# lms-07/LGTEUN

Measured on AMD Instinct MI355X. Metric: train image-pairs/sec, GF-2 4-band 128x128, K=4, bs=32/GPU, higher is better.
Workload: dtype f32 (GEMMs and the local mixer: split 16-bit MFMA -- f16 pairs in the forward FFN, the W2 products of its backward and P V, bf16 triples elsewhere -- fp32 accumulate; fp32-equivalent); 1 GPU; BASELINE configs[1]: C=4, MS 32x32, PAN 128x128, K=4, 32 pairs/GPU, train step = fwd + L1 + bwd + Adam + StepLR tick; mode=faithful, global_batch=32, parallelism=dp1, dropout=True

## Files before the change

### include/lgteun_hip.h

```cpp
#ifndef LGTEUN_HIP_H
#define LGTEUN_HIP_H

#include <stddef.h>
#include <stdint.h>

#ifdef __cplusplus
extern "C" {
#endif

#define LG_TENSORS_SHARED 12
#define LG_TENSORS_PER_STAGE 119

#define LG_FLAG_FAITHFUL 1
#define LG_FLAG_SAVE 2
#define LG_FLAG_DROPOUT 4

#define LG_FLAG_BWD_LGT 8
#define LG_FLAG_BWD_DATA 16

#define LG_FLAG_CHAINED 32

#define LG_FLAG_DEFER_DEAD 64

#define LG_FLAG_STAGEWISE 128
// ... 10 lines not shown
    int32_t precision;
    uint32_t variant;
} lg_config;

#define LG_VAR_FFN_IMPL_MASK 3u
#define LG_VAR_FFN_STRIP 1u
#define LG_VAR_FFN_SAVE_MASK (3u << 2)
#define LG_VAR_FFN_SAVE3 (1u << 2)
#define LG_VAR_FFN_SAVE5 (2u << 2)
#define LG_VAR_FFN_BWD32_PAIR (1u << 4)
#define LG_VAR_FFN_DWBWD_TILE (1u << 5)
#define LG_VAR_ATTN_BWD_R3 (1u << 6)
#define LG_VAR_DSTEP_TILES (1u << 7)
#define LG_VAR_ATTN_FWD_VALU (1u << 8)
#define LG_VAR_FFN_BF16X3 (1u << 9)
#define LG_VAR_FFT_FULL (1u << 10)
#define LG_VAR_FFN_BWD_BF16X3 (1u << 11)
#define LG_VAR_ATTN_BWD_CORE_M (1u << 12)
#define LG_VAR_FFN_XS (1u << 13)
#define LG_VAR_ATTN_BF16X3 (1u << 14)
#define LG_VAR_FFN_H3_RECOMPUTE (1u << 15)
#define LG_VAR_ATTN_BWD_RESTATS (1u << 16)
#define LG_VAR_REDUCE_PER_BLOCK (1u << 17)
#define LG_VAR_ALL 0x3ffffu

typedef struct lg_plan lg_plan;

const char* lg_version(void);
#define LG_ABI_VERSION 2
int32_t lg_abi_version(void);
const char* lg_last_error(void);

int lg_plan_create(const lg_config* cfg, const int64_t* offsets, int32_t n_offsets, lg_plan** out);
void lg_plan_destroy(lg_plan* plan);
int lg_plan_describe(const lg_plan* plan, char* buf, size_t n);
size_t lg_workspace_bytes(const lg_plan* plan, int32_t B, int32_t train);

int lgteun_forward(const lg_plan* plan, const float* params, const float* ms, const float* pan, float* out,
                   void* workspace, size_t workspace_bytes, int32_t B, int32_t flags, uint64_t seed, void* stream);

int lgteun_dead_forward(const lg_plan* plan, const float* params, void* workspace, size_t workspace_bytes, int32_t B, int32_t flags,
                        uint64_t seed, void* stream);

int lgteun_backward(const lg_plan* plan, const float* params, float* grads, const float* ms, const float* pan,
                    const float* dout, void* workspace, size_t workspace_bytes, int32_t B, int32_t flags,
                    uint64_t seed, void* stream);

// ... 103 lines not shown
```

### lgteun_amd/_lib.py

```python
import ctypes
import os
from ctypes import POINTER, c_char_p, c_double, c_float, c_int32, c_int64, c_size_t, c_uint64, c_void_p

_HERE = os.path.dirname(os.path.abspath(__file__))
LIB_PATH = os.environ.get('LGTEUN_HIP_LIB') or os.path.join(_HERE, '_lgteun_hip.so')

LG_FLAG_FAITHFUL = 1
LG_FLAG_SAVE = 2
LG_FLAG_DROPOUT = 4
LG_FLAG_BWD_LGT = 8
LG_FLAG_BWD_DATA = 16
LG_FLAG_CHAINED = 32
LG_FLAG_DEFER_DEAD = 64
LG_FLAG_STAGEWISE = 128
KERNEL_IDS = {n: i for i, n in enumerate(['none', 'ffn1', 'ffn', 'fft', 'attn', 'upfuse', 'down', 'embed', 'tail', 'datastep', 'ffn1_bwd',
                                           'ffn2_bwd', 'fft_bwd', 'attn_bwd', 'wgrad', 'batch', 'scene_gather', 'scene_blend'])}


class LgConfig(ctypes.Structure):
    _fields_ = [('C', c_int32), ('K', c_int32), ('H', c_int32), ('W', c_int32), ('precision', c_int32), ('variant', ctypes.c_uint32)]


LG_VAR_FFN_STRIP = 1
LG_VAR_FFN_SAVE3, LG_VAR_FFN_SAVE5 = 1 << 2, 2 << 2
LG_VAR_FFN_BWD32_PAIR, LG_VAR_FFN_DWBWD_TILE, LG_VAR_ATTN_BWD_R3 = 1 << 4, 1 << 5, 1 << 6
LG_VAR_DSTEP_TILES = 1 << 7
LG_VAR_ATTN_FWD_VALU = 1 << 8
LG_VAR_FFN_BF16X3 = 1 << 9
LG_VAR_FFT_FULL = 1 << 10
LG_VAR_FFN_BWD_BF16X3 = 1 << 11
LG_VAR_ATTN_BWD_CORE_M = 1 << 12
LG_VAR_FFN_XS = 1 << 13
LG_VAR_ATTN_BF16X3 = 1 << 14
LG_VAR_FFN_H3_RECOMPUTE = 1 << 15
LG_VAR_ATTN_BWD_RESTATS = 1 << 16
LG_VAR_REDUCE_PER_BLOCK = 1 << 17
LG_OPT_ADAM, LG_OPT_ADAMW, LG_OPT_SGD, LG_OPT_RMSPROP = 0, 1, 2, 3
LG_OPT_AMSGRAD, LG_OPT_NESTEROV, LG_OPT_CENTERED = 1, 2, 4
LG_DT_U8, LG_DT_U16, LG_DT_F32 = 0, 1, 2
LG_ABI_VERSION = 2


def variant_from_env(env=None):
    env = os.environ if env is None else env
    v = {'strip': LG_VAR_FFN_STRIP, 'tile': 2, 'xp': 3}.get(env.get('LG_FFN_IMPL', ''), 0)
    v |= {'3': LG_VAR_FFN_SAVE3, '5': LG_VAR_FFN_SAVE5}.get(env.get('LG_FFN_SAVE', ''), 0)
    if env.get('LG_FFN_BWD32') == 'pair':
        v |= LG_VAR_FFN_BWD32_PAIR
    if env.get('LG_FFN_DWBWD') == 'tile':
        v |= LG_VAR_FFN_DWBWD_TILE
    if env.get('LG_ATTN_BWD') in ('old', 'r3'):
        v |= LG_VAR_ATTN_BWD_R3
    if env.get('LG_DSTEP') == 'tiles':
        v |= LG_VAR_DSTEP_TILES
    if env.get('LG_ATTN_FWD', '') == 'valu':
        v |= LG_VAR_ATTN_FWD_VALU
    if env.get('LG_FFN_SPLIT', '') == 'bf16x3':
        v |= LG_VAR_FFN_BF16X3
    if env.get('LG_FFT', '') == 'full':
        v |= LG_VAR_FFT_FULL
    if env.get('LG_FFN_BWD_SPLIT', '') == 'bf16x3':
        v |= LG_VAR_FFN_BWD_BF16X3
    if env.get('LG_ATTN_BWD_CORE', '') == 'm':
        v |= LG_VAR_ATTN_BWD_CORE_M
    if env.get('LG_FFN_FWD', '') == 'xs':
        v |= LG_VAR_FFN_XS
    if env.get('LG_ATTN_SPLIT', '') == 'bf16x3':
        v |= LG_VAR_ATTN_BF16X3
    if env.get('LG_FFN_H3', '') == 'recompute':
        v |= LG_VAR_FFN_H3_RECOMPUTE
    if env.get('LG_ATTN_BWD_STATS', '') == 'recompute':
        v |= LG_VAR_ATTN_BWD_RESTATS
    if env.get('LG_REDUCE', '') == 'per_block':
        v |= LG_VAR_REDUCE_PER_BLOCK
    return v


class LgteunHipError(RuntimeError):
    pass


_lib = None

SIGNATURES = {
    'lg_version': (c_char_p, []),
    'lg_abi_version': (c_int32, []),
    'lg_last_error': (c_char_p, []),
    'lg_plan_create': (c_int32, [POINTER(LgConfig), POINTER(c_int64), c_int32, POINTER(c_void_p)]),
    'lg_plan_destroy': (None, [c_void_p]),
    'lg_plan_describe': (c_int32, [c_void_p, c_char_p, c_size_t]),
    'lg_workspace_bytes': (c_size_t, [c_void_p, c_int32, c_int32]),
    'lgteun_forward': (c_int32, [c_void_p, c_void_p, c_void_p, c_void_p, c_void_p, c_void_p, c_size_t, c_int32, c_int32,
                                 c_uint64, c_void_p]),
    'lgteun_backward': (c_int32, [c_void_p, c_void_p, c_void_p, c_void_p, c_void_p, c_void_p, c_void_p, c_size_t, c_int32,
                                  c_int32, c_uint64, c_void_p]),
    'lgteun_dead_forward': (c_int32, [c_void_p, c_void_p, c_void_p, c_size_t, c_int32, c_int32, c_uint64, c_void_p]),
    'lg_l1_loss': (c_int32, [c_void_p, c_void_p, c_void_p, c_void_p, c_int64, c_int64, c_float, c_void_p]),
# ... 76 lines not shown
```

### lgteun_amd/csrc/bwd_kernels.h

```cpp
#pragma once
#include "common.h"

struct WgradArgs {
    const void* Y;
    const void* X;
    float* dW;
    float* db;
    long P;
    int ldy, ldx, ldw;
    int N, K;
    int n_valid, k_valid;
    int ybf, xbf;
    int xgelu;
};
size_t wgrad_slab_floats(int N, int K, long P);
#define PIXEL_PART_WGS 2048
size_t chan_partial_floats(int C, int B, int H, int W);
struct ChanReduce {
    float* dst[14];
    float* dst2[14];
    int stride[14];
    int NK, C, nslices;
    unsigned allc_mask;
};
// ... 107 lines not shown
int launch_tail_bwd(int C, const TailBwdArgs& a, hipStream_t s);

struct EmbedBwdArgs {
    const float* dx;
    const float* z;
    float* dz;
    const float *dww, *dwb, *w, *b, *lng;
    float *d_dww, *d_dwb, *d_lng, *d_lnb;
    float *d_w, *d_b;
    float* part;
    int HW;
    long total;
};
size_t embed_bwd_part_floats(int C);
int launch_embed_bwd(int C, const EmbedBwdArgs& a, hipStream_t s);

struct DownBwdArgs {
    const float* dy;
    float* du;
    const float* dskip;
    float* dx;
    const float* w;
    int B, H, W;
};
int launch_down_bwd_a(int E, const DownBwdArgs& a, hipStream_t s);
int launch_down_bwd_b(int E, const DownBwdArgs& a, hipStream_t s);

struct UpFuseBwdArgs {
    const float* dy;
    float* dt;
    float* dskip;
    float* v;
    float* dxb;
    float* tmp;
    const float *fw, *upw;
    int B, H, W;
};
int launch_upfuse_bwd_a(int E, const UpFuseBwdArgs& a, hipStream_t s);
int launch_upfuse_bwd_b(int E, const UpFuseBwdArgs& a, hipStream_t s);

struct FfnDwBwdArgs {
    const float* dy;
    const void* g3;
    const void* h2;
    void* dh2;
    int hbf;
    int pre;
    const float *w3t;
    const float* dww;
    float *slab_w, *slab_b;
    float *d_dww, *d_dwb;
    int B, h, w;
};
size_t ffn_dw_bwd_slab_floats(int e, int B, int h, int w);
int launch_ffn_dw_bwd(int e, const FfnDwBwdArgs& a, hipStream_t s);
struct Ffn1BwdArgs {
    const void* dh2;
    const void* g1;
    const float* x;
    const float* dy;
    void* dh1;
    float* y2;
// ... 183 lines not shown
```

### lgteun_amd/csrc/k_bwd.hip

```cpp
#include <string.h>

#include "kernels.h"
#include "bwd_kernels.h"
#include "backward.h"

struct BwdBufs {
    float *dzA, *dzB, *gu3, *gs1, *gu1, *gr, *gd3, *gt1, *gd1;
    float *dx[3];
    float *dh2, *dh1, *y2, *do2, *dg, *dym, *cat, *y1, *dqkv;
    float *w3t[5], *w2t[5], *w1t[5], *wsp, *dt, *dskip, *v, *du, *fft_scratch;
    float* slab_arena;
    float* attn_stats;
    float* ffn_scales;
    size_t slab_cap;
    ReduceQueue rq;
    size_t bytes;
};

static size_t dpos_slab_floats() {
    const size_t f = (size_t)ATTN_BWD_F_WGS * ATTN_BWD_F_ROW, r3 = (size_t)512 * 2 * 64 * 64;
    return f > r3 ? f : r3;
}
static void carve_bwd(const lg_plan* plan, int B, void* base, BwdBufs& bb) {
    const lg_config& c = plan->cfg;
// ... 297 lines not shown
    d.part = bb.rq.take(chan_partial_floats(c.C, B, H, W));
    if (!d.part) return -3;
    RC(launch_dw_bwd(0, d, s));
    RC(launch_resample_adj(0, bb.gd1, dz, planes, H, W, 1, s));
    return bb.rq.block_end();
}

static int lgt_bwd(const lg_plan* pl, const float* P, float* G, int st, const NetBufs& nb, BwdBufs& bb, const float* dout,
                   const float* zin, int B, int flags, uint64_t seed, hipStream_t s) {
    const lg_config& c = pl->cfg;
    const int E = 4 * c.C;
    const long P0 = (long)B * c.H * c.W, P1 = P0 / 4;
    const float* posT = nb.posT + (size_t)st * 5 * 2 * 64 * 64;
    float *A = bb.dx[0], *Bf = bb.dx[1], *Cf = bb.dx[2];
    RC(ffn_transposes(pl, P, st, 0, 5, nb, bb, s));
    TailBwdArgs tb;
    tb.dout = dout; tb.x = nb.blk[4].xout; tb.dx = A; tb.dz = bb.dzA; tb.w = P + pl->lgt(st, L_TAILW);
    tb.d_w = G + pl->lgt(st, L_TAILW); tb.d_b = G + pl->lgt(st, L_TAILB);
    tb.HW = c.H * c.W; tb.total = P0; tb.part = bb.rq.take(tail_bwd_part_floats(c.C));
    if (!tb.part) return -3;
    RC(launch_tail_bwd(c.C, tb, s));
    RC(block_bwd(pl, P, G, st, 4, nb.blk[4], bb, posT + 4 * 8192, A, Bf, Cf, B, flags, seed, s));
    RC(block_bwd(pl, P, G, st, 3, nb.blk[3], bb, posT + 3 * 8192, Cf, Bf, A, B, flags, seed, s));
    UpFuseBwdArgs ub;
    ub.dy = A; ub.dt = bb.dt; ub.dskip = bb.dskip; ub.v = bb.v; ub.dxb = Bf; ub.tmp = Cf;
    ub.fw = P + pl->lgt(st, L_FUSEW); ub.upw = P + pl->lgt(st, L_UPW);
    ub.B = B; ub.H = c.H; ub.W = c.W;
    RC(launch_upfuse_bwd_a(E, ub, s));
    RC(wgrad(A, E, nb.t_up, E, G + pl->lgt(st, L_FUSEW), 2 * E, G + pl->lgt(st, L_FUSEB), P0, E, E, E, E, 0, 0, bb, s));
    RC(wgrad(A, E, nb.blk[1].xout, E, G + pl->lgt(st, L_FUSEW) + E, 2 * E, nullptr, P0, E, E, E, E, 0, 0, bb, s));
    RC(launch_upfuse_bwd_b(E, ub, s));
    RC(wgrad(bb.v, E, nb.blk[2].xout, 2 * E, G + pl->lgt(st, L_UPW), 2 * E, G + pl->lgt(st, L_UPB), P1, E, 2 * E, E, 2 * E, 0, 0, bb, s));
    RC(block_bwd(pl, P, G, st, 2, nb.blk[2], bb, posT + 2 * 8192, Bf, Cf, A, B, flags, seed, s));
    DownBwdArgs db;
    db.dy = A; db.du = bb.du; db.dskip = bb.dskip; db.dx = Bf; db.w = P + pl->lgt(st, L_DOWNW);
    db.B = B; db.H = c.H; db.W = c.W;
    RC(launch_down_bwd_a(E, db, s));
    RC(wgrad(A, 2 * E, nb.u_down, E, G + pl->lgt(st, L_DOWNW), E, G + pl->lgt(st, L_DOWNB), P1, 2 * E, E, 2 * E, E, 0, 0, bb, s));
    RC(launch_down_bwd_b(E, db, s));
    RC(block_bwd(pl, P, G, st, 1, nb.blk[1], bb, posT + 1 * 8192, Bf, Cf, A, B, flags, seed, s));
    RC(block_bwd(pl, P, G, st, 0, nb.blk[0], bb, posT + 0 * 8192, A, Bf, Cf, B, flags, seed, s));
    EmbedBwdArgs eb;
    eb.dx = Cf; eb.z = zin; eb.dz = bb.dzA;
    eb.dww = P + pl->lgt(st, L_PE_DWW); eb.dwb = P + pl->lgt(st, L_PE_DWB); eb.w = P + pl->lgt(st, L_PE_W); eb.b = P + pl->lgt(st, L_PE_B);
    eb.lng = P + pl->lgt(st, L_PE_LNG);
    eb.d_dww = G + pl->lgt(st, L_PE_DWW); eb.d_dwb = G + pl->lgt(st, L_PE_DWB);
    eb.d_lng = G + pl->lgt(st, L_PE_LNG); eb.d_lnb = G + pl->lgt(st, L_PE_LNB);
    eb.d_w = G + pl->lgt(st, L_PE_W); eb.d_b = G + pl->lgt(st, L_PE_B);
    eb.HW = c.H * c.W; eb.total = P0; eb.part = bb.rq.take(embed_bwd_part_floats(c.C));
    if (!eb.part) return -3;
    RC(launch_embed_bwd(c.C, eb, s));
    return 0;
}

int op_data_step_bwd(const lg_plan* pl, const float* P, float* G, int st, NetBufs& nb, void* bwd_ws, const float* z_in, const float* pan,
                     const float* g, float* dz, int B, hipStream_t s) {
    BwdBufs bb;
    carve_bwd(pl, B, bwd_ws, bb);
    ReduceQueueScope rqs(bb, s, pl->route.reduce_per_block);
    const int rc = data_step_bwd(pl, P, G, st, nb, bb, z_in, pan, g, dz, B, s);
    const int rc2 = reduce_queue_end();
// ... 51 lines not shown
```

### lgteun_amd/csrc/k_bwd_pixel.hip

```cpp
#include <string.h>

#include "kernels.h"
#include "bwd_kernels.h"
#include "resample_tile.h"

template <int N>
__device__ __forceinline__ float block_sum(float (&v)[N], float* sm ) {
    const int wave = threadIdx.x >> 6, lane = threadIdx.x & 63;
#pragma unroll
    for (int i = 0; i < N; ++i) {
        float s = v[i];
#pragma unroll
        for (int off = 32; off > 0; off >>= 1) s += __shfl_xor(s, off);
        if (lane == 0) sm[wave * N + i] = s;
    }
    __syncthreads();
    float r = 0.f;
    if (threadIdx.x < N) r = sm[threadIdx.x] + sm[N + threadIdx.x] + sm[2 * N + threadIdx.x] + sm[3 * N + threadIdx.x];
    __syncthreads();
    return r;
}

template <int MODE>
__global__ __launch_bounds__(256) void k_resample_adj(const float* __restrict__ gout, float* __restrict__ gin, int hi, int wi, int ho, int wo,
                                                      int accumulate, int rt, int grows) {
    constexpr int NC = AdjPlan<MODE>::NC, PL = NC + 1;
    extern __shared__ float sm[];
// ... 515 lines not shown
    const int ix = (int)(p % a.W);
    const long r = p / a.W;
    const int iy = (int)(r % a.H);
    const long b = r / a.H;
    const int ho = a.H / 2, wo = a.W / 2;
    AdjPlan<0> py, px;
    py.make(iy, a.H, ho);
    px.make(ix, a.W, wo);
    float4 acc = *reinterpret_cast<const float4*>(a.dskip + p * E + 4 * q);
#pragma unroll
    for (int ya = 0; ya < 3; ++ya) {
        const int yy = clampi(py.base + ya, 0, ho - 1);
#pragma unroll
        for (int xb = 0; xb < 3; ++xb) {
            const int xx = clampi(px.base + xb, 0, wo - 1);
            const float wgt = py.coef[ya] * px.coef[xb];
            const float4 v = *reinterpret_cast<const float4*>(a.du + ((b * ho + yy) * (long)wo + xx) * E + 4 * q);
            acc.x += wgt * v.x; acc.y += wgt * v.y; acc.z += wgt * v.z; acc.w += wgt * v.w;
        }
    }
    *reinterpret_cast<float4*>(a.dx + p * E + 4 * q) = acc;
}

int launch_down_bwd_a(int E, const DownBwdArgs& a, hipStream_t s) {
    long total = (long)a.B * (a.H / 2) * (a.W / 2);
    int grid = (int)((total + 255) / 256);
    if (E == 16) k_down_bwd_a<16><<<grid, 256, 0, s>>>(a);
    else if (E == 32) k_down_bwd_a<32><<<grid, 256, 0, s>>>(a);
    else { lg_set_error("down_bwd: E=%d unsupported", E); return -1; }
    LG_CHECK_LAUNCH();
    return 0;
}
int launch_down_bwd_b(int E, const DownBwdArgs& a, hipStream_t s) {
    long total = (long)a.B * a.H * a.W;
    const int ppw = 256 / (E / 4);
    int grid = (int)((total + ppw - 1) / ppw);
    if (E == 16) k_down_bwd_b<16><<<grid, 256, 0, s>>>(a);
    else if (E == 32) k_down_bwd_b<32><<<grid, 256, 0, s>>>(a);
    else { lg_set_error("down_bwd: E=%d unsupported", E); return -1; }
    LG_CHECK_LAUNCH();
    return 0;
}

template <int E>
__global__ __launch_bounds__(256) void k_upfuse_bwd_a(UpFuseBwdArgs a) {
    constexpr int LPP = E / 4, PPW = 256 / LPP, LDU = E + 4;
    __shared__ float sFw[E * 2 * E];
    __shared__ __attribute__((aligned(16))) float dx_[PPW * LDU];
    lds_stage(sFw, a.fw, E * 2 * E);
    __syncthreads();
    const int q = threadIdx.x % LPP, slot = threadIdx.x / LPP;
    const long total = (long)a.B * a.H * a.W;
    for (long p = (long)blockIdx.x * PPW + slot; p < total; p += (long)gridDim.x * PPW) {
        *reinterpret_cast<float4*>(dx_ + slot * LDU + 4 * q) = *reinterpret_cast<const float4*>(a.dy + p * E + 4 * q);
// ... 78 lines not shown
    __builtin_amdgcn_wave_barrier();
    __builtin_amdgcn_fence(__ATOMIC_ACQUIRE, "wavefront");
    float v[E];
#pragma unroll
    for (int k = 0; k < E / 4; ++k) {
        const float4 t = *reinterpret_cast<const float4*>(vx + slot * LDU + 4 * k);
        v[4 * k] = t.x; v[4 * k + 1] = t.y; v[4 * k + 2] = t.z; v[4 * k + 3] = t.w;
    }
    float o[NO];
#pragma unroll
    for (int j = 0; j < NO; ++j) {
        float acc = 0.f;
#pragma unroll
        for (int n = 0; n < E; ++n) acc += sUw[n * 2 * E + NO * q + j] * v[n];
        o[j] = acc;
    }
    if (pv) {
        float4* dxo = reinterpret_cast<float4*>(a.dxb + p * 2 * E + NO * q);
        dxo[0] = make_float4(o[0], o[1], o[2], o[3]);
        dxo[1] = make_float4(o[4], o[5], o[6], o[7]);
    }
}

int launch_upfuse_bwd_a(int E, const UpFuseBwdArgs& a, hipStream_t s) {
    if (E != 16 && E != 32) { lg_set_error("upfuse_bwd: E=%d unsupported", E); return -1; }
    const long total = (long)a.B * a.H * a.W;
    const int ppw = 256 / (E / 4);
    if (total % ppw) { lg_set_error("upfuse_bwd: %ld pixels are not a multiple of %d", total, ppw); return -2; }
    const long ng = total / ppw;
    const int grid = (int)(ng < 2048 ? ng : 2048);
    if (E == 16) k_upfuse_bwd_a<16><<<grid, 256, 0, s>>>(a);
    else k_upfuse_bwd_a<32><<<grid, 256, 0, s>>>(a);
    LG_CHECK_LAUNCH();
    return 0;
}
int launch_upfuse_bwd_b(int E, const UpFuseBwdArgs& a, hipStream_t s) {
    if (!a.tmp) { lg_set_error("upfuse_bwd: row-contracted scratch missing"); return -2; }
    if (E != 16 && E != 32) { lg_set_error("upfuse_bwd: E=%d unsupported", E); return -1; }
    const int ppw = 256 / (E / 4), wi = a.W / 2;
    const int rows = a.B * a.H;
    dim3 gh((wi + ppw - 1) / ppw, rows < 1024 ? rows : 1024);
    if (E == 16) k_upadj_h<16><<<gh, 256, 0, s>>>(a.dt, a.tmp, rows, a.W);
    else k_upadj_h<32><<<gh, 256, 0, s>>>(a.dt, a.tmp, rows, a.W);
    LG_CHECK_LAUNCH();
    const long total = (long)a.B * (a.H / 2) * wi;
    const int grid = (int)((total + ppw - 1) / ppw);
    if (E == 16) k_upfuse_bwd_b<16><<<grid, 256, 0, s>>>(a);
    else k_upfuse_bwd_b<32><<<grid, 256, 0, s>>>(a);
    LG_CHECK_LAUNCH();
    return 0;
}
```

### lgteun_amd/csrc/mfma.h

```cpp
#pragma once
#include <hip/hip_runtime.h>

typedef float f32x4 __attribute__((ext_vector_type(4)));

template <int MT, int NT, int K>
__device__ __forceinline__ void wave_gemm(f32x4 (&acc)[MT][NT], const float* A, int lda, const float* __restrict__ Wg) {
    const int lane = threadIdx.x & 63, r = lane & 15, g = lane >> 4;
#pragma unroll 2
    for (int k0 = 0; k0 < K; k0 += 16) {
        float4 av[MT], bv[NT];
#pragma unroll
        for (int mt = 0; mt < MT; ++mt) av[mt] = *reinterpret_cast<const float4*>(A + (mt * 16 + r) * lda + k0 + 4 * g);
#pragma unroll
        for (int nt = 0; nt < NT; ++nt) bv[nt] = *reinterpret_cast<const float4*>(Wg + (size_t)(nt * 16 + r) * K + k0 + 4 * g);
#pragma unroll
        for (int ks = 0; ks < 4; ++ks)
#pragma unroll
            for (int mt = 0; mt < MT; ++mt)
#pragma unroll
                for (int nt = 0; nt < NT; ++nt) {
                    const float a_ = ks == 0 ? av[mt].x : (ks == 1 ? av[mt].y : (ks == 2 ? av[mt].z : av[mt].w));
                    const float b_ = ks == 0 ? bv[nt].x : (ks == 1 ? bv[nt].y : (ks == 2 ? bv[nt].z : bv[nt].w));
                    acc[mt][nt] = __builtin_amdgcn_mfma_f32_16x16x4f32(a_, b_, acc[mt][nt], 0, 0, 0);
                }
// ... 32 lines not shown
#pragma unroll
        for (int kb = 0; kb < KB; ++kb) bf[nt][kb] = *reinterpret_cast<const float4*>(Wg + (size_t)(nt * 16 + r) * K + kb * 16 + 4 * g);
}
template <int MT, int NT, int KB>
__device__ __forceinline__ void wave_gemm_rb(f32x4 (&acc)[MT][NT], const float* A, int lda, const float4 (&bf)[NT][KB]) {
    const int lane = threadIdx.x & 63, r = lane & 15, g = lane >> 4;
#pragma unroll
    for (int kb = 0; kb < KB; ++kb) {
        float4 av[MT];
#pragma unroll
        for (int mt = 0; mt < MT; ++mt) av[mt] = *reinterpret_cast<const float4*>(A + (mt * 16 + r) * lda + kb * 16 + 4 * g);
#pragma unroll
        for (int ks = 0; ks < 4; ++ks)
#pragma unroll
            for (int mt = 0; mt < MT; ++mt)
#pragma unroll
                for (int nt = 0; nt < NT; ++nt) {
                    const float a_ = ks == 0 ? av[mt].x : (ks == 1 ? av[mt].y : (ks == 2 ? av[mt].z : av[mt].w));
                    const float b_ = ks == 0 ? bf[nt][kb].x : (ks == 1 ? bf[nt][kb].y : (ks == 2 ? bf[nt][kb].z : bf[nt][kb].w));
                    acc[mt][nt] = __builtin_amdgcn_mfma_f32_16x16x4f32(a_, b_, acc[mt][nt], 0, 0, 0);
                }
    }
}
```

### lgteun_amd/csrc/route.h

```cpp
#pragma once
#include <stddef.h>
#include "../../include/lgteun_hip.h"

enum FfnFwdKernel {
    FFN_FWD_XR,
    FFN_FWD_XS,
    FFN_FWD_X32,
    FFN_FWD_X64,
    FFN_FWD_STRIP,
    FFN_FWD_TILE,
    FFN_FWD_UNFUSED
};
enum FfnArith { FFN_ARITH_F32, FFN_ARITH_BF16, FFN_ARITH_F16X2, FFN_ARITH_BF16X3 };
enum FfnSlot { FFN_SLOT_A1 = 1, FFN_SLOT_G1 = 2, FFN_SLOT_H2 = 4, FFN_SLOT_A3 = 8, FFN_SLOT_G3 = 16 };
enum FfnDwBwdKernel { FFN_DWBWD_XS, FFN_DWBWD_H, FFN_DWBWD_TILE };
enum Ffn1BwdKernel { FFN1_BWD_XS, FFN1_BWD_X32, FFN1_BWD_TILE };

struct FfnRoute {
    int e, h, w;
    FfnFwdKernel fwd[2];
    FfnArith arith;
    bool hbf;
    bool scales;
    int wsplit_np;
// ... 3 lines not shown
    FfnDwBwdKernel dw;
    Ffn1BwdKernel px;
    bool bwd_scales;
    bool wgrad_w2, wgrad_w1, wgrad_w3;
};

enum AttnFwdKernel { ATTN_FWD_M, ATTN_FWD_VALU };
enum AttnBwdKernel { ATTN_BWD_F, ATTN_BWD_R3, ATTN_BWD_R3_CORE_M };
struct MixerRoute {
    int e;
    AttnFwdKernel fwd;
    bool bf16;
    bool f16x2;
    bool stats;
    AttnBwdKernel bwd;
};

struct LgRoute {
    FfnRoute ffn[2];
    MixerRoute mix[2];
    bool dstep_fused;
    bool fft_full;
    bool reduce_per_block;
};

int lg_resolve_route(const lg_config& cfg, LgRoute* r);
int lg_describe_route(const lg_config& cfg, const LgRoute& r, char* buf, size_t n);
```

### lgteun_amd/csrc/route.hip

```cpp
#include <stdio.h>

#include "kernels.h"
#include "bwd_kernels.h"

static void resolve_ffn(const lg_config& cfg, int e, int h, int w, FfnRoute& f) {
    const uint32_t v = cfg.variant;
    const int impl = (int)(v & LG_VAR_FFN_IMPL_MASK);
    const uint32_t sv = v & LG_VAR_FFN_SAVE_MASK;
    const bool split = impl == 0;
    const bool strips = (h & 7) == 0 && (w & 15) == 0;
    f.e = e; f.h = h; f.w = w;
    f.hbf = cfg.precision == 1 && e != 64;
    f.scales = cfg.precision == 0 && split && !(v & LG_VAR_FFN_BF16X3);
    f.arith = !split ? FFN_ARITH_F32 : f.hbf ? FFN_ARITH_BF16 : f.scales ? FFN_ARITH_F16X2 : FFN_ARITH_BF16X3;
    f.wsplit_np = e < 32 ? 0 : f.hbf ? 1 : f.scales ? 2 : 3;

    const int save_form = (e != 16 || !split) ? 5 : sv == LG_VAR_FFN_SAVE5 ? 5 : (sv == LG_VAR_FFN_SAVE3 ? (cfg.precision == 0 ? 3 : 5) : 2);
    f.pre = save_form != 5;
    f.px = (e == 16 && save_form == 2) || (e == 32 && split && !(v & LG_VAR_FFN_BWD32_PAIR)) ? FFN1_BWD_XS : (e == 32 && split) ? FFN1_BWD_X32 : FFN1_BWD_TILE;
    const bool dw_tile = (v & LG_VAR_FFN_DWBWD_TILE) && !(e == 16 && f.hbf);
    f.dw = ((e == 16 && save_form == 2) || (e == 32 && split)) && !dw_tile && strips ? FFN_DWBWD_XS : FFN_DWBWD_TILE;
    const bool xr_built = split && !(v & LG_VAR_FFN_XS) && (f.hbf || f.scales);
    if (e == 16 && f.dw == FFN_DWBWD_XS && (v & LG_VAR_FFN_H3_RECOMPUTE) && xr_built && !f.hbf) f.dw = FFN_DWBWD_H;
    f.bwd_scales = f.px == FFN1_BWD_XS && f.dw != FFN_DWBWD_TILE && f.scales && !(v & LG_VAR_FFN_BWD_BF16X3);
// ... 21 lines not shown
    const uint32_t v = cfg.variant;
    m.e = e;
    m.fwd = (v & LG_VAR_ATTN_FWD_VALU) ? ATTN_FWD_VALU : ATTN_FWD_M;
    m.bf16 = cfg.precision == 1;
    m.f16x2 = cfg.precision == 0 && m.fwd == ATTN_FWD_M && !(v & LG_VAR_ATTN_BF16X3) && !(v & LG_VAR_FFN_IMPL_MASK) && !(v & LG_VAR_FFN_BF16X3);
    m.bwd = (attn_bwd_fused(e) && !(v & LG_VAR_ATTN_BWD_R3)) ? ATTN_BWD_F : (e == 32 && (v & LG_VAR_ATTN_BWD_CORE_M)) ? ATTN_BWD_R3_CORE_M : ATTN_BWD_R3;
    m.stats = cfg.precision == 0 && m.fwd == ATTN_FWD_M && !(v & LG_VAR_ATTN_BWD_RESTATS) && m.bwd != ATTN_BWD_R3_CORE_M;
}

int lg_resolve_route(const lg_config& cfg, LgRoute* r) {
    const uint32_t v = cfg.variant;
    if (v & ~LG_VAR_ALL) { lg_set_error("plan_create: unknown variant bits 0x%x", v & ~LG_VAR_ALL); return -2; }
    if ((v & LG_VAR_FFN_SAVE_MASK) == LG_VAR_FFN_SAVE_MASK) { lg_set_error("plan_create: invalid FFN save variant"); return -2; }
    if ((v & LG_VAR_FFN_IMPL_MASK) > LG_VAR_FFN_STRIP) { lg_set_error("plan_create: FFN implementation field (LG_VAR_FFN_IMPL_MASK) = %u: only 0 and LG_VAR_FFN_STRIP exist", v & LG_VAR_FFN_IMPL_MASK); return -2; }
    if (cfg.precision == 1 && (v & LG_VAR_FFN_IMPL_MASK)) { lg_set_error("plan_create: FFN implementation field (LG_VAR_FFN_IMPL_MASK): LG_VAR_FFN_STRIP is an fp32 kernel set, precision = 1 has none"); return -2; }
    const int E = 4 * cfg.C;
    resolve_ffn(cfg, E, cfg.H, cfg.W, r->ffn[0]);
    resolve_ffn(cfg, 2 * E, cfg.H / 2, cfg.W / 2, r->ffn[1]);
    resolve_mixer(cfg, E, r->mix[0]);
    resolve_mixer(cfg, 2 * E, r->mix[1]);
    r->dstep_fused = !(v & LG_VAR_DSTEP_TILES) && dstep_fused_ok(cfg.C, cfg.H, cfg.W);
    r->fft_full = (v & LG_VAR_FFT_FULL) != 0;
    r->reduce_per_block = (v & LG_VAR_REDUCE_PER_BLOCK) != 0;
    return 0;
}

static const char* slots_text(unsigned slots, bool a1_pre, bool a3_pre, char (&buf)[48]) {
    int n = 0;
    buf[0] = 0;
    auto add = [&](unsigned bit, const char* name) { if (slots & bit) n += snprintf(buf + n, sizeof(buf) - n, "%s%s", n ? "," : "", name); };
    add(FFN_SLOT_A1, a1_pre ? "a1:h1" : "a1"); add(FFN_SLOT_G1, "g1"); add(FFN_SLOT_H2, "h2"); add(FFN_SLOT_A3, a3_pre ? "a3:h3" : "a3"); add(FFN_SLOT_G3, "g3");
    return n ? buf : "-";
}

int lg_describe_route(const lg_config& cfg, const LgRoute& r, char* buf, size_t n) {
    static const char* const fwd_names[] = {"k_ffn_xr", "k_ffn_xs", "k_ffn_x32", "k_ffn1_x64+k_ffn2_x64", "k_ffn_strip", "k_ffn_fused", "k_ffn1+k_ffn2"};
    static const char* const arith_names[] = {"f32", "bf16", "f16x2", "bf16x3"};
    static const char* const dw_names[] = {"k_ffn_dw_bwd_xs", "k_ffn_dw_bwd_h", "k_ffn_dw_bwd"};
    static const char* const px_names[] = {"k_ffn1_bwd_xs", "k_ffn1_bwd_x32", "k_ffn1_bwd"};
    static const char* const attn_bwd_names[] = {"k_attn_bwd_f", "k_attn_bwd_core+k_attn_bwd_epi", "k_attn_bwd_core_m+k_attn_bwd_epi"};
    size_t off = 0;
    bool full = false;
    auto put = [&](const char* fmt, auto... a) {
        const int k = snprintf(buf + off, n - off, fmt, a...);
        if (k < 0 || (size_t)k >= n - off) full = true; else off += (size_t)k;
    };
// ... 28 lines not shown
```

Measured before the change: 6553 image-pairs/sec.

## Fuse weight-gradient reductions into LGT transition backward kernels (down, upfuse)

Adds fused backward kernels for the LGT down-sampling and up/fuse transitions. Each kernel computes the data gradient and also accumulates the conv weight and bias gradients per workgroup with fp32 MFMA outer products, then a slab reduction sums the partials. This replaces separate wgrad launches that re-read dy and the conv inputs from global memory. The fused path is the default, the old split path stays behind an env flag, and the cost is extra slab scratch and more complex kernels with wave-level barriers.

Result: no change. 6599 image-pairs/sec, median of 6 (+0.7%).

```diff
diff --git a/include/lgteun_hip.h b/include/lgteun_hip.h
--- a/include/lgteun_hip.h
+++ b/include/lgteun_hip.h
@@ -56,7 +56,8 @@
 #define LG_VAR_FFN_H3_RECOMPUTE (1u << 15)
 #define LG_VAR_ATTN_BWD_RESTATS (1u << 16)
 #define LG_VAR_REDUCE_PER_BLOCK (1u << 17)
-#define LG_VAR_ALL 0x3ffffu
+#define LG_VAR_LGT_TRANS_SPLIT (1u << 21)
+#define LG_VAR_ALL 0x23ffffu
 
 typedef struct lg_plan lg_plan;
 
diff --git a/lgteun_amd/_lib.py b/lgteun_amd/_lib.py
--- a/lgteun_amd/_lib.py
+++ b/lgteun_amd/_lib.py
@@ -35,6 +35,7 @@
 LG_VAR_FFN_H3_RECOMPUTE = 1 << 15
 LG_VAR_ATTN_BWD_RESTATS = 1 << 16
 LG_VAR_REDUCE_PER_BLOCK = 1 << 17
+LG_VAR_LGT_TRANS_SPLIT = 1 << 21
 LG_OPT_ADAM, LG_OPT_ADAMW, LG_OPT_SGD, LG_OPT_RMSPROP = 0, 1, 2, 3
 LG_OPT_AMSGRAD, LG_OPT_NESTEROV, LG_OPT_CENTERED = 1, 2, 4
 LG_DT_U8, LG_DT_U16, LG_DT_F32 = 0, 1, 2
@@ -73,6 +74,8 @@
         v |= LG_VAR_ATTN_BWD_RESTATS
     if env.get('LG_REDUCE', '') == 'per_block':
         v |= LG_VAR_REDUCE_PER_BLOCK
+    if env.get('LG_LGT_TRANS_BWD', '') == 'split':
+        v |= LG_VAR_LGT_TRANS_SPLIT
     return v
 
 
diff --git a/lgteun_amd/csrc/bwd_kernels.h b/lgteun_amd/csrc/bwd_kernels.h
--- a/lgteun_amd/csrc/bwd_kernels.h
+++ b/lgteun_amd/csrc/bwd_kernels.h
@@ -153,8 +153,12 @@
     float* dx;
     const float* w;
     int B, H, W;
-};
+    const float* u = nullptr;
+    float* slab = nullptr;
+};
+size_t trans_bwd_slab_floats(int E);
 int launch_down_bwd_a(int E, const DownBwdArgs& a, hipStream_t s);
+int launch_down_bwd_aw(int E, const DownBwdArgs& a, float* d_w, float* d_b, hipStream_t s);
 int launch_down_bwd_b(int E, const DownBwdArgs& a, hipStream_t s);
 
 struct UpFuseBwdArgs {
@@ -166,9 +170,16 @@
     float* tmp;
     const float *fw, *upw;
     int B, H, W;
+    const float* t_up = nullptr;
+    const float* skip = nullptr;
+    const float* xb = nullptr;
+    float* slab = nullptr;
 };
 int launch_upfuse_bwd_a(int E, const UpFuseBwdArgs& a, hipStream_t s);
 int launch_upfuse_bwd_b(int E, const UpFuseBwdArgs& a, hipStream_t s);
+bool upfuse_bwd_rows_ok(int E, int W);
+int launch_upfuse_bwd_ar(int E, const UpFuseBwdArgs& a, float* d_w, float* d_b, hipStream_t s);
+int launch_upfuse_bwd_bw(int E, const UpFuseBwdArgs& a, int upadj, float* d_w, float* d_b, hipStream_t s);
 
 struct FfnDwBwdArgs {
     const float* dy;
diff --git a/lgteun_amd/csrc/k_bwd.hip b/lgteun_amd/csrc/k_bwd.hip
--- a/lgteun_amd/csrc/k_bwd.hip
+++ b/lgteun_amd/csrc/k_bwd.hip
@@ -343,21 +343,43 @@
     RC(launch_tail_bwd(c.C, tb, s));
     RC(block_bwd(pl, P, G, st, 4, nb.blk[4], bb, posT + 4 * 8192, A, Bf, Cf, B, flags, seed, s));
     RC(block_bwd(pl, P, G, st, 3, nb.blk[3], bb, posT + 3 * 8192, Cf, Bf, A, B, flags, seed, s));
+    const bool fused = !pl->route.lgt_trans_split;
+    const bool rows_ok = fused && upfuse_bwd_rows_ok(E, c.W);
     UpFuseBwdArgs ub;
     ub.dy = A; ub.dt = bb.dt; ub.dskip = bb.dskip; ub.v = bb.v; ub.dxb = Bf; ub.tmp = Cf;
     ub.fw = P + pl->lgt(st, L_FUSEW); ub.upw = P + pl->lgt(st, L_UPW);
     ub.B = B; ub.H = c.H; ub.W = c.W;
-    RC(launch_upfuse_bwd_a(E, ub, s));
-    RC(wgrad(A, E, nb.t_up, E, G + pl->lgt(st, L_FUSEW), 2 * E, G + pl->lgt(st, L_FUSEB), P0, E, E, E, E, 0, 0, bb, s));
-    RC(wgrad(A, E, nb.blk[1].xout, E, G + pl->lgt(st, L_FUSEW) + E, 2 * E, nullptr, P0, E, E, E, E, 0, 0, bb, s));
-    RC(launch_upfuse_bwd_b(E, ub, s));
-    RC(wgrad(bb.v, E, nb.blk[2].xout, 2 * E, G + pl->lgt(st, L_UPW), 2 * E, G + pl->lgt(st, L_UPB), P1, E, 2 * E, E, 2 * E, 0, 0, bb, s));
+    ub.t_up = nb.t_up; ub.skip = nb.blk[1].xout; ub.xb = nb.blk[2].xout;
+    if (rows_ok) {
+        ub.slab = bb.rq.take(trans_bwd_slab_floats(E));
+        if (!ub.slab) return -3;
+        RC(launch_upfuse_bwd_ar(E, ub, G + pl->lgt(st, L_FUSEW), G + pl->lgt(st, L_FUSEB), s));
+    } else {
+        RC(launch_upfuse_bwd_a(E, ub, s));
+        RC(wgrad(A, E, nb.t_up, E, G + pl->lgt(st, L_FUSEW), 2 * E, G + pl->lgt(st, L_FUSEB), P0, E, E, E, E, 0, 0, bb, s));
+        RC(wgrad(A, E, nb.blk[1].xout, E, G + pl->lgt(st, L_FUSEW) + E, 2 * E, nullptr, P0, E, E, E, E, 0, 0, bb, s));
+    }
+    if (fused) {
+        ub.slab = bb.rq.take(trans_bwd_slab_floats(E));
+        if (!ub.slab) return -3;
+        RC(launch_upfuse_bwd_bw(E, ub, rows_ok ? 0 : 1, G + pl->lgt(st, L_UPW), G + pl->lgt(st, L_UPB), s));
+    } else {
+        RC(launch_upfuse_bwd_b(E, ub, s));
+        RC(wgrad(bb.v, E, nb.blk[2].xout, 2 * E, G + pl->lgt(st, L_UPW), 2 * E, G + pl->lgt(st, L_UPB), P1, E, 2 * E, E, 2 * E, 0, 0, bb, s));
+    }
     RC(block_bwd(pl, P, G, st, 2, nb.blk[2], bb, posT + 2 * 8192, Bf, Cf, A, B, flags, seed, s));
     DownBwdArgs db;
     db.dy = A; db.du = bb.du; db.dskip = bb.dskip; db.dx = Bf; db.w = P + pl->lgt(st, L_DOWNW);
     db.B = B; db.H = c.H; db.W = c.W;
-    RC(launch_down_bwd_a(E, db, s));
-    RC(wgrad(A, 2 * E, nb.u_down, E, G + pl->lgt(st, L_DOWNW), E, G + pl->lgt(st, L_DOWNB), P1, 2 * E, E, 2 * E, E, 0, 0, bb, s));
+    if (fused) {
+        db.u = nb.u_down;
+        db.slab = bb.rq.take(trans_bwd_slab_floats(E));
+        if (!db.slab) return -3;
+        RC(launch_down_bwd_aw(E, db, G + pl->lgt(st, L_DOWNW), G + pl->lgt(st, L_DOWNB), s));
+    } else {
+        RC(launch_down_bwd_a(E, db, s));
+        RC(wgrad(A, 2 * E, nb.u_down, E, G + pl->lgt(st, L_DOWNW), E, G + pl->lgt(st, L_DOWNB), P1, 2 * E, E, 2 * E, E, 0, 0, bb, s));
+    }
     RC(launch_down_bwd_b(E, db, s));
     RC(block_bwd(pl, P, G, st, 1, nb.blk[1], bb, posT + 1 * 8192, Bf, Cf, A, B, flags, seed, s));
     RC(block_bwd(pl, P, G, st, 0, nb.blk[0], bb, posT + 0 * 8192, A, Bf, Cf, B, flags, seed, s));
diff --git a/lgteun_amd/csrc/k_bwd_pixel.hip b/lgteun_amd/csrc/k_bwd_pixel.hip
--- a/lgteun_amd/csrc/k_bwd_pixel.hip
+++ b/lgteun_amd/csrc/k_bwd_pixel.hip
@@ -3,6 +3,7 @@
 #include "kernels.h"
 #include "bwd_kernels.h"
 #include "resample_tile.h"
+#include "mfma.h"
 
 template <int N>
 __device__ __forceinline__ float block_sum(float (&v)[N], float* sm ) {
@@ -564,6 +565,76 @@
     *reinterpret_cast<float4*>(a.dx + p * E + 4 * q) = acc;
 }
 
+
+#define TRANS_BWD_WGS 512
+__device__ __forceinline__ float4 keep4(bool keep, const float4& v) { return make_float4(keep ? v.x : 0.f, keep ? v.y : 0.f, keep ? v.z : 0.f, keep ? v.w : 0.f); }
+struct DownAwOps { float4 y0, y1, x0; };
+template <int E>
+__device__ __forceinline__ DownAwOps down_aw_fetch(const DownBwdArgs& a, long p, long total, int q) {
+    const long pc_ = p < total ? p : total - 1;
+    DownAwOps o;
+    o.y0 = *reinterpret_cast<const float4*>(a.dy + pc_ * 2 * E + 8 * q);
+    o.y1 = *reinterpret_cast<const float4*>(a.dy + pc_ * 2 * E + 8 * q + 4);
+    o.x0 = *reinterpret_cast<const float4*>(a.u + pc_ * E + 4 * q);
+    return o;
+}
+template <int E>
+__global__ __launch_bounds__(256) void k_down_bwd_aw(DownBwdArgs a) {
+    constexpr int LPP = E / 4, PPW = 256 / LPP, PY = px_pitch(2 * E), PX = px_pitch(E), MT = 2 * E / 16, NT = E / 16;
+    constexpr int IMG = PPW * (PY + PX), SCR = 4 * wave_pixel_row<MT, NT>();
+    __shared__ float sW[2 * E * E];
+    __shared__ __attribute__((aligned(16))) float sm[IMG > SCR ? IMG : SCR];
+    float* yi = sm;
+    float* xi = sm + PPW * PY;
+    lds_stage(sW, a.w, 2 * E * E);
+    __syncthreads();
+    const int q = threadIdx.x % LPP, slot = threadIdx.x / LPP, wave = threadIdx.x >> 6;
+    const long total = (long)a.B * (a.H / 2) * (a.W / 2);
+    const long ngroups = (total + PPW - 1) / PPW;
+    f32x4 acc[MT][NT];
+    float bsum[MT];
+#pragma unroll
+    for (int mt = 0; mt < MT; ++mt) {
+        bsum[mt] = 0.f;
+#pragma unroll
+        for (int nt = 0; nt < NT; ++nt) acc[mt][nt] = f32x4{0.f, 0.f, 0.f, 0.f};
+    }
+    DownAwOps nx = down_aw_fetch<E>(a, blockIdx.x * (long)PPW + slot, total, q);
+    for (long grp = blockIdx.x; grp < ngroups; grp += gridDim.x) {
+        const long p = grp * PPW + slot;
+        const bool pv = p < total;
+        *reinterpret_cast<float4*>(yi + slot * PY + 8 * q) = keep4(pv, nx.y0);
+        *reinterpret_cast<float4*>(yi + slot * PY + 8 * q + 4) = keep4(pv, nx.y1);
+        *reinterpret_cast<float4*>(xi + slot * PX + 4 * q) = keep4(pv, nx.x0);
+        nx = down_aw_fetch<E>(a, p + (long)gridDim.x * PPW, total, q);
+        __builtin_amdgcn_fence(__ATOMIC_RELEASE, "wavefront");
+        __builtin_amdgcn_wave_barrier();
+        __builtin_amdgcn_fence(__ATOMIC_ACQUIRE, "wavefront");
+        float dy[2 * E];
+#pragma unroll
+        for (int k = 0; k < 2 * E / 4; ++k) {
+            const float4 v = *reinterpret_cast<const float4*>(yi + slot * PY + 4 * k);
+            dy[4 * k] = v.x; dy[4 * k + 1] = v.y; dy[4 * k + 2] = v.z; dy[4 * k + 3] = v.w;
+        }
+        float v[4];
+#pragma unroll
+        for (int u = 0; u < 4; ++u) {
+            float s_ = 0.f;
+#pragma unroll
+            for (int n = 0; n < 2 * E; ++n) s_ += sW[n * E + q * 4 + u] * dy[n];
+            v[u] = s_;
+        }
+        if (pv) *reinterpret_cast<float4*>(a.du + p * E + 4 * q) = make_float4(v[0], v[1], v[2], v[3]);
+        const int w0 = wave * (PPW / 4);
+        wave_pixel_outer<MT, NT>(acc, bsum, yi + w0 * PY, PY, xi + w0 * PX, PX, 0, PPW / 16, 1);
+        __builtin_amdgcn_fence(__ATOMIC_RELEASE, "wavefront");
+        __builtin_amdgcn_wave_barrier();
+        __builtin_amdgcn_fence(__ATOMIC_ACQUIRE, "wavefront");
+    }
+    __syncthreads();
+    wave_pixel_outer_store<MT, NT>(acc, bsum, sm, a.slab + (size_t)blockIdx.x * (2 * E * E), a.slab + (size_t)gridDim.x * (2 * E * E) + (size_t)blockIdx.x * 2 * E);
+}
+
 int launch_down_bwd_a(int E, const DownBwdArgs& a, hipStream_t s) {
     long total = (long)a.B * (a.H / 2) * (a.W / 2);
     int grid = (int)((total + 255) / 256);
@@ -572,6 +643,19 @@
     else { lg_set_error("down_bwd: E=%d unsupported", E); return -1; }
     LG_CHECK_LAUNCH();
     return 0;
+}
+size_t trans_bwd_slab_floats(int E) { return (size_t)TRANS_BWD_WGS * ((size_t)2 * E * E + 2 * E); }
+int launch_down_bwd_aw(int E, const DownBwdArgs& a, float* d_w, float* d_b, hipStream_t s) {
+    if (!a.u || !a.slab || !d_w || !d_b) { lg_set_error("down_bwd: conv input / partial-sum scratch / destinations missing"); return -2; }
+    if (E != 16 && E != 32) { lg_set_error("down_bwd: E=%d unsupported", E); return -1; }
+    const long total = (long)a.B * (a.H / 2) * (a.W / 2);
+    const int ppw = 256 / (E / 4);
+    const long ng = (total + ppw - 1) / ppw;
+    const int grid = (int)(ng < TRANS_BWD_WGS ? ng : TRANS_BWD_WGS);
+    if (E == 16) k_down_bwd_aw<16><<<grid, 256, 0, s>>>(a);
+    else k_down_bwd_aw<32><<<grid, 256, 0, s>>>(a);
+    LG_CHECK_LAUNCH();
+    return launch_reduce_slab_wb(a.slab, a.slab + (size_t)grid * 2 * E * E, grid, 2 * E, E, d_w, E, d_b, s);
 }
 int launch_down_bwd_b(int E, const DownBwdArgs& a, hipStream_t s) {
     long total = (long)a.B * a.H * a.W;
@@ -696,6 +780,193 @@
     }
 }
 
+
+#define UPFUSE_AR_F4 4
+__device__ __forceinline__ void upfuse_ar_fetch(const UpFuseBwdArgs& a, long o, int nq, f32x4 (&ry)[UPFUSE_AR_F4], f32x4 (&rt)[UPFUSE_AR_F4],
+                                                f32x4 (&rs)[UPFUSE_AR_F4]) {
+#pragma unroll
+    for (int k = 0; k < UPFUSE_AR_F4; ++k) {
+        const int i = k * 256 + (int)threadIdx.x;
+        const long j = o + 4L * (i < nq ? i : nq - 1);
+        ry[k] = *reinterpret_cast<const f32x4*>(a.dy + j);
+        rt[k] = *reinterpret_cast<const f32x4*>(a.t_up + j);
+        rs[k] = *reinterpret_cast<const f32x4*>(a.skip + j);
+    }
+}
+template <int E>
+__global__ __launch_bounds__(256) void k_upfuse_bwd_ar(UpFuseBwdArgs a) {
+    constexpr int LPP = E / 4, PY = px_pitch(E), PX = px_pitch(2 * E), PD = E + 4, MT = E / 16, NT = 2 * E / 16, PL = 11;
+    extern __shared__ __attribute__((aligned(16))) float smr[];
+    const int W = a.W, wi = W / 2, nq = W * LPP;
+    float* sFw = smr;
+    float* yi = sFw + E * 2 * E;
+    float* xi = yi + W * PY;
+    float* di = xi + W * PX;
+    float* spx = di + W * PD;
+    lds_stage(sFw, a.fw, E * 2 * E);
+    for (int i = threadIdx.x; i < wi; i += 256) {
+        AdjPlan<1> pl;
+        pl.make(i, wi, W);
+        spx[i * PL] = __int_as_float(pl.base);
+#pragma unroll
+        for (int k = 0; k < 10; ++k) spx[i * PL + 1 + k] = pl.coef[k];
+    }
+    const int wave = threadIdx.x >> 6;
+    const long rows = (long)a.B * a.H;
+    f32x4 acc[MT][NT];
+    float bsum[MT];
+#pragma unroll
+    for (int mt = 0; mt < MT; ++mt) {
+        bsum[mt] = 0.f;
+#pragma unroll
+        for (int nt = 0; nt < NT; ++nt) acc[mt][nt] = f32x4{0.f, 0.f, 0.f, 0.f};
+    }
+    f32x4 ry[UPFUSE_AR_F4], rt[UPFUSE_AR_F4], rs[UPFUSE_AR_F4];
+    upfuse_ar_fetch(a, (long)blockIdx.x * W * E, nq, ry, rt, rs);
+    for (long row = blockIdx.x; row < rows; row += gridDim.x) {
+#pragma unroll
+        for (int k = 0; k < UPFUSE_AR_F4; ++k) {
+            const int i = k * 256 + (int)threadIdx.x;
+            if (i < nq) {
+                const int p = i / LPP, q = i - p * LPP;
+                *reinterpret_cast<f32x4*>(yi + p * PY + 4 * q) = ry[k];
+                *reinterpret_cast<f32x4*>(xi + p * PX + 4 * q) = rt[k];
+                *reinterpret_cast<f32x4*>(xi + p * PX + E + 4 * q) = rs[k];
+            }
+        }
+        __syncthreads();
+        upfuse_ar_fetch(a, (row + gridDim.x < rows ? row + gridDim.x : row) * W * E, nq, ry, rt, rs);
+        for (int i = threadIdx.x; i < nq; i += 256) {
+            const int p = i / LPP, q = i - p * LPP;
+            float dy[E];
+#pragma unroll
+            for (int k = 0; k < E / 4; ++k) {
+                const float4 v = *reinterpret_cast<const float4*>(yi + p * PY + 4 * k);
+                dy[4 * k] = v.x; dy[4 * k + 1] = v.y; dy[4 * k + 2] = v.z; dy[4 * k + 3] = v.w;
+            }
+            float v[4] = {0.f, 0.f, 0.f, 0.f}, w[4] = {0.f, 0.f, 0.f, 0.f};
+#pragma unroll
+            for (int n = 0; n < E; ++n) {
+                const float4 f1 = *reinterpret_cast<const float4*>(sFw + n * 2 * E + 4 * q);
+                const float4 f2 = *reinterpret_cast<const float4*>(sFw + n * 2 * E + E + 4 * q);
+                v[0] += f1.x * dy[n]; v[1] += f1.y * dy[n]; v[2] += f1.z * dy[n]; v[3] += f1.w * dy[n];
+                w[0] += f2.x * dy[n]; w[1] += f2.y * dy[n]; w[2] += f2.z * dy[n]; w[3] += f2.w * dy[n];
+            }
+            *reinterpret_cast<float4*>(di + p * PD + 4 * q) = make_float4(v[0], v[1], v[2], v[3]);
+            *reinterpret_cast<float4*>(a.dskip + (row * W + p) * E + 4 * q) = make_float4(w[0], w[1], w[2], w[3]);
+        }
+        wave_pixel_outer<MT, NT>(acc, bsum, yi, PY, xi, PX, wave, W / 4, 4);
+        __syncthreads();
+        for (int i = threadIdx.x; i < wi * LPP; i += 256) {
+            const int ix = i / LPP, q = i - ix * LPP;
+            const float* pp = spx + ix * PL;
+            const int bx = __float_as_int(pp[0]);
+            float4 o = make_float4(0.f, 0.f, 0.f, 0.f);
+#pragma unroll
+            for (int k = 0; k < 10; ++k) {
+                const int x = clampi(bx + k, 0, W - 1);
+                const float4 v = *reinterpret_cast<const float4*>(di + x * PD + 4 * q);
+                const float c = pp[1 + k];
+                o.x += c * v.x; o.y += c * v.y; o.z += c * v.z; o.w += c * v.w;
+            }
+            *reinterpret_cast<float4*>(a.tmp + (row * wi + ix) * E + 4 * q) = o;
+        }
+        __syncthreads();
+    }
+    wave_pixel_outer_store<MT, NT>(acc, bsum, smr, a.slab + (size_t)blockIdx.x * (2 * E * E), a.slab + (size_t)gridDim.x * (2 * E * E) + (size_t)blockIdx.x * E);
+}
+
+struct UpfuseBwOps { float4 tap[10], x0, x1; AdjPlan<1> py; };
+template <int E>
+__device__ __forceinline__ UpfuseBwOps upfuse_bw_fetch(const UpFuseBwdArgs& a, long p, long total, int q) {
+    const int hi = a.H / 2, wi = a.W / 2;
+    const long pc_ = p < total ? p : 0;
+    const int ix = (int)(pc_ % wi);
+    const long r = pc_ / wi;
+    const int iy = (int)(r % hi);
+    const long b = r / hi;
+    UpfuseBwOps o;
+    o.py.make(iy, hi, a.H);
+    const float* __restrict__ src = a.tmp + ((b * a.H) * (long)wi + ix) * E + 4 * q;
+#pragma unroll
+    for (int k = 0; k < 10; ++k) {
+        const int y = clampi(o.py.base + k, 0, a.H - 1);
+        o.tap[k] = *reinterpret_cast<const float4*>(src + (long)y * wi * E);
+    }
+    o.x0 = *reinterpret_cast<const float4*>(a.xb + pc_ * 2 * E + 8 * q);
+    o.x1 = *reinterpret_cast<const float4*>(a.xb + pc_ * 2 * E + 8 * q + 4);
+    return o;
+}
+template <int E>
+__global__ __launch_bounds__(256) void k_upfuse_bwd_bw(UpFuseBwdArgs a) {
+    constexpr int LPP = E / 4, PPW = 256 / LPP, NO = 2 * E / LPP, PY = px_pitch(E), PX = px_pitch(2 * E), MT = E / 16, NT = 2 * E / 16;
+    static_assert(NO == 8, "eight outputs per lane");
+    constexpr int IMG = PPW * (PY + PX), SCR = 4 * wave_pixel_row<MT, NT>();
+    __shared__ float sUw[E * 2 * E];
+    __shared__ __attribute__((aligned(16))) float sm[IMG > SCR ? IMG : SCR];
+    float* vx = sm;
+    float* xi = sm + PPW * PY;
+    lds_stage(sUw, a.upw, E * 2 * E);
+    __syncthreads();
+    const int q = threadIdx.x % LPP, slot = threadIdx.x / LPP, wave = threadIdx.x >> 6;
+    const int hi = a.H / 2, wi = a.W / 2;
+    const long total = (long)a.B * hi * wi;
+    const long ngroups = (total + PPW - 1) / PPW;
+    f32x4 acc[MT][NT];
+    float bsum[MT];
+#pragma unroll
+    for (int mt = 0; mt < MT; ++mt) {
+        bsum[mt] = 0.f;
+#pragma unroll
+        for (int nt = 0; nt < NT; ++nt) acc[mt][nt] = f32x4{0.f, 0.f, 0.f, 0.f};
+    }
+    UpfuseBwOps nx = upfuse_bw_fetch<E>(a, blockIdx.x * (long)PPW + slot, total, q);
+    for (long grp = blockIdx.x; grp < ngroups; grp += gridDim.x) {
+        const long p = grp * PPW + slot;
+        const bool pv = p < total;
+        float4 v4 = make_float4(0.f, 0.f, 0.f, 0.f);
+#pragma unroll
+        for (int k = 0; k < 10; ++k) {
+            const float4 t = nx.tap[k];
+            const float c = nx.py.coef[k];
+            v4.x += c * t.x; v4.y += c * t.y; v4.z += c * t.z; v4.w += c * t.w;
+        }
+        *reinterpret_cast<float4*>(vx + slot * PY + 4 * q) = keep4(pv, v4);
+        *reinterpret_cast<float4*>(xi + slot * PX + NO * q) = keep4(pv, nx.x0);
+        *reinterpret_cast<float4*>(xi + slot * PX + NO * q + 4) = keep4(pv, nx.x1);
+        nx = upfuse_bw_fetch<E>(a, p + (long)gridDim.x * PPW, total, q);
+        __builtin_amdgcn_fence(__ATOMIC_RELEASE, "wavefront");
+        __builtin_amdgcn_wave_barrier();
+        __builtin_amdgcn_fence(__ATOMIC_ACQUIRE, "wavefront");
+        float v[E];
+#pragma unroll
+        for (int k = 0; k < E / 4; ++k) {
+            const float4 t = *reinterpret_cast<const float4*>(vx + slot * PY + 4 * k);
+            v[4 * k] = t.x; v[4 * k + 1] = t.y; v[4 * k + 2] = t.z; v[4 * k + 3] = t.w;
+        }
+        float o[NO];
+#pragma unroll
+        for (int j = 0; j < NO; ++j) {
+            float s_ = 0.f;
+#pragma unroll
+            for (int n = 0; n < E; ++n) s_ += sUw[n * 2 * E + NO * q + j] * v[n];
+            o[j] = s_;
+        }
+        if (pv) {
+            float4* dxo = reinterpret_cast<float4*>(a.dxb + p * 2 * E + NO * q);
+            dxo[0] = make_float4(o[0], o[1], o[2], o[3]);
+            dxo[1] = make_float4(o[4], o[5], o[6], o[7]);
+        }
+        const int w0 = wave * (PPW / 4);
+        wave_pixel_outer<MT, NT>(acc, bsum, vx + w0 * PY, PY, xi + w0 * PX, PX, 0, PPW / 16, 1);
+        __builtin_amdgcn_fence(__ATOMIC_RELEASE, "wavefront");
+        __builtin_amdgcn_wave_barrier();
+        __builtin_amdgcn_fence(__ATOMIC_ACQUIRE, "wavefront");
+    }
+    __syncthreads();
+    wave_pixel_outer_store<MT, NT>(acc, bsum, sm, a.slab + (size_t)blockIdx.x * (2 * E * E), a.slab + (size_t)gridDim.x * (2 * E * E) + (size_t)blockIdx.x * E);
+}
+
 int launch_upfuse_bwd_a(int E, const UpFuseBwdArgs& a, hipStream_t s) {
     if (E != 16 && E != 32) { lg_set_error("upfuse_bwd: E=%d unsupported", E); return -1; }
     const long total = (long)a.B * a.H * a.W;
@@ -724,3 +995,44 @@
     LG_CHECK_LAUNCH();
     return 0;
 }
+
+static size_t upfuse_ar_lds(int E, int W) {
+    const size_t img = (size_t)E * 2 * E + (size_t)W * (px_pitch(E) + px_pitch(2 * E) + E + 4) + (size_t)(W / 2) * 11;
+    const size_t scr = (size_t)4 * (2 * E * E + E);
+    return (img > scr ? img : scr) * sizeof(float);
+}
+bool upfuse_bwd_rows_ok(int E, int W) {
+    return (E == 16 || E == 32) && W % 4 == 0 && W * (E / 4) <= 256 * UPFUSE_AR_F4 && upfuse_ar_lds(E, W) <= 150 * 1024;
+}
+int launch_upfuse_bwd_ar(int E, const UpFuseBwdArgs& a, float* d_w, float* d_b, hipStream_t s) {
+    if (!a.tmp || !a.t_up || !a.skip || !a.slab || !d_w || !d_b) { lg_set_error("upfuse_bwd: conv inputs / scratch / destinations missing"); return -2; }
+    if (!upfuse_bwd_rows_ok(E, a.W)) { lg_set_error("upfuse_bwd: rows of %d pixels at E=%d have no row-owning instance", a.W, E); return -2; }
+    static DeviceOnce attr_once;
+    if (int rc = lds_attr_once(attr_once, "upfuse_bwd", 150 * 1024, k_upfuse_bwd_ar<16>, k_upfuse_bwd_ar<32>)) return rc;
+    const long rows = (long)a.B * a.H;
+    const int grid = (int)(rows < TRANS_BWD_WGS ? rows : TRANS_BWD_WGS);
+    const size_t lds = upfuse_ar_lds(E, a.W);
+    if (E == 16) k_upfuse_bwd_ar<16><<<grid, 256, lds, s>>>(a);
+    else k_upfuse_bwd_ar<32><<<grid, 256, lds, s>>>(a);
+    LG_CHECK_LAUNCH();
+    return launch_reduce_slab_wb(a.slab, a.slab + (size_t)grid * 2 * E * E, grid, E, 2 * E, d_w, 2 * E, d_b, s);
+}
+int launch_upfuse_bwd_bw(int E, const UpFuseBwdArgs& a, int upadj, float* d_w, float* d_b, hipStream_t s) {
+    if (!a.tmp || !a.xb || !a.slab || !d_w || !d_b) { lg_set_error("upfuse_bwd: conv input / scratch / destinations missing"); return -2; }
+    if (E != 16 && E != 32) { lg_set_error("upfuse_bwd: E=%d unsupported", E); return -1; }
+    const int ppw = 256 / (E / 4), wi = a.W / 2;
+    if (upadj) {
+        const int rows = a.B * a.H;
+        dim3 gh((wi + ppw - 1) / ppw, rows < 1024 ? rows : 1024);
+        if (E == 16) k_upadj_h<16><<<gh, 256, 0, s>>>(a.dt, a.tmp, rows, a.W);
+        else k_upadj_h<32><<<gh, 256, 0, s>>>(a.dt, a.tmp, rows, a.W);
+        LG_CHECK_LAUNCH();
+    }
+    const long total = (long)a.B * (a.H / 2) * wi;
+    const long ng = (total + ppw - 1) / ppw;
+    const int grid = (int)(ng < TRANS_BWD_WGS ? ng : TRANS_BWD_WGS);
+    if (E == 16) k_upfuse_bwd_bw<16><<<grid, 256, 0, s>>>(a);
+    else k_upfuse_bwd_bw<32><<<grid, 256, 0, s>>>(a);
+    LG_CHECK_LAUNCH();
+    return launch_reduce_slab_wb(a.slab, a.slab + (size_t)grid * 2 * E * E, grid, E, 2 * E, d_w, 2 * E, d_b, s);
+}
diff --git a/lgteun_amd/csrc/mfma.h b/lgteun_amd/csrc/mfma.h
--- a/lgteun_amd/csrc/mfma.h
+++ b/lgteun_amd/csrc/mfma.h
@@ -78,3 +78,51 @@
                 }
     }
 }
+
+constexpr int px_pitch(int n) { return (n & 31) == 16 ? n : n + 16; }
+
+template <int MT, int NT>
+__device__ __forceinline__ void wave_pixel_outer(f32x4 (&acc)[MT][NT], float (&bsum)[MT], const float* Y, int ldy, const float* X, int ldx, int s0,
+                                                 int ns, int ds) {
+    const int lane = threadIdx.x & 63, r = lane & 15, g = lane >> 4;
+    for (int s = s0; s < ns; s += ds) {
+        const int p = 4 * s + g;
+        float av[MT], bv[NT];
+#pragma unroll
+        for (int mt = 0; mt < MT; ++mt) av[mt] = Y[p * ldy + mt * 16 + r];
+#pragma unroll
+        for (int nt = 0; nt < NT; ++nt) bv[nt] = X[p * ldx + nt * 16 + r];
+#pragma unroll
+        for (int mt = 0; mt < MT; ++mt) {
+            bsum[mt] += av[mt];
+#pragma unroll
+            for (int nt = 0; nt < NT; ++nt) acc[mt][nt] = __builtin_amdgcn_mfma_f32_16x16x4f32(av[mt], bv[nt], acc[mt][nt], 0, 0, 0);
+        }
+    }
+}
+
+template <int MT, int NT>
+constexpr int wave_pixel_row() { return MT * NT * 256 + MT * 16; }
+template <int MT, int NT>
+__device__ __forceinline__ void wave_pixel_outer_store(const f32x4 (&acc)[MT][NT], const float (&bsum)[MT], float* scr, float* __restrict__ wrow,
+                                                       float* __restrict__ brow) {
+    constexpr int N = 16 * NT, NW = MT * NT * 256, ROW = wave_pixel_row<MT, NT>();
+    const int wave = threadIdx.x >> 6, lane = threadIdx.x & 63, r = lane & 15, g = lane >> 4;
+    float* my = scr + wave * ROW;
+#pragma unroll
+    for (int mt = 0; mt < MT; ++mt) {
+#pragma unroll
+        for (int nt = 0; nt < NT; ++nt)
+#pragma unroll
+            for (int i = 0; i < 4; ++i) my[(mt * 16 + 4 * g + i) * N + nt * 16 + r] = acc[mt][nt][i];
+        float b = bsum[mt];
+        b += __shfl_xor(b, 16);
+        b += __shfl_xor(b, 32);
+        if (g == 0) my[NW + mt * 16 + r] = b;
+    }
+    __syncthreads();
+    for (int i = threadIdx.x; i < ROW; i += 256) {
+        const float v = (scr[i] + scr[ROW + i]) + (scr[2 * ROW + i] + scr[3 * ROW + i]);
+        if (i < NW) wrow[i] = v; else brow[i - NW] = v;
+    }
+}
diff --git a/lgteun_amd/csrc/route.h b/lgteun_amd/csrc/route.h
--- a/lgteun_amd/csrc/route.h
+++ b/lgteun_amd/csrc/route.h
@@ -49,6 +49,7 @@
     bool dstep_fused;
     bool fft_full;
     bool reduce_per_block;
+    bool lgt_trans_split;
 };
 
 int lg_resolve_route(const lg_config& cfg, LgRoute* r);
diff --git a/lgteun_amd/csrc/route.hip b/lgteun_amd/csrc/route.hip
--- a/lgteun_amd/csrc/route.hip
+++ b/lgteun_amd/csrc/route.hip
@@ -67,6 +67,7 @@
     r->dstep_fused = !(v & LG_VAR_DSTEP_TILES) && dstep_fused_ok(cfg.C, cfg.H, cfg.W);
     r->fft_full = (v & LG_VAR_FFT_FULL) != 0;
     r->reduce_per_block = (v & LG_VAR_REDUCE_PER_BLOCK) != 0;
+    r->lgt_trans_split = (v & LG_VAR_LGT_TRANS_SPLIT) != 0;
     return 0;
 }
 
```
